# InternetMaximalism/plonky2_bn254

Hardware: AMD Instinct MI355X
Metric: G1 scalar-mul STARK proofs/sec (256-bit scalars) (higher is better)
Workload: dtype u64 (Goldilocks p = 2^64-2^32+1; BN254 Fq as 10x26-bit Montgomery limbs); 1 GPU; configs[1]: batch of 1024 G1 scalar-muls on 1 GPU per step = 8 proofs x 128 instances, 2^16 rows, W=781, standard_fast_config; instances_per_proof=128, steps_in_flight=4, parallelism=1 GPU, no collective

## Files before the change

### plonky2_bn254_amd/csrc/aux.h

```cpp
#pragma once
#include "gl_dev.h"
#include "../../include/bn254_stark.h"

static constexpr int CTL_MAX = 2, CTL_MAX_COLS = 160;

struct CtlSpecDev {
  int ncols[CTL_MAX];
  int filter_col[CTL_MAX];
  short col_start[CTL_MAX][CTL_MAX_COLS];
  unsigned char col_bits[CTL_MAX][CTL_MAX_COLS];
};

struct StarkShape {
  int W = 0;
  int rc_begin = 0, rc_end = 0;
  int table_col = 0, freq_col = 0;
  int n_ctl = 2;
  int n_constraints = 0;
  CtlSpecDev ctl;
  GL_HD int n_rc() const { return rc_end - rc_begin; }
  GL_HD int n_helpers() const { return (n_rc() + 1) / 2; }
  GL_HD int n_aux() const { return 2 * (n_helpers() + 1) + 2 * n_ctl; }
  GL_HD int n_lookup_cols() const { return 2 * (n_helpers() + 1); }
  GL_HD int n_total_constraints() const { return n_constraints + 2 * (n_helpers() + 2) + 2 * 2 * n_ctl; }
};

size_t aux_scratch_words(const StarkShape& sh, size_t N);
void aux_build(const StarkShape& sh, const u64* d_trace, size_t N, const u64 betas[2], const u64 gammas[2], u64* d_aux,
               u64* d_scratch, int* d_err, hipStream_t st);
```

### plonky2_bn254_amd/csrc/aux.hip

```cpp
#include <algorithm>
#include "aux.h"

static constexpr int LOGUP_SPAN = 16;
static constexpr int LOGUP_INV_BATCH = 4;

__global__ __launch_bounds__(256) void k_logup_inv_table(u64 beta0, u64 beta1, u64* __restrict__ inv) {
  const u32 t = blockIdx.x * blockDim.x + threadIdx.x;
  if (t >= 2 * 65536 / LOGUP_INV_BATCH) return;
  u64 d[LOGUP_INV_BATCH], pre[LOGUP_INV_BATCH];
  u64 acc = 1;
#pragma unroll
  for (int j = 0; j < LOGUP_INV_BATCH; j++) {
    const u64 x = gl_add((j & 1) ? beta1 : beta0, (u64)(2 * t + (j >> 1)));
    d[j] = x ? x : 1;
    pre[j] = acc;
    acc = gl_mul(acc, d[j]);
  }
  u64 r = gl_inv(acc);
  u64 o[LOGUP_INV_BATCH];
#pragma unroll
  for (int j = LOGUP_INV_BATCH - 1; j >= 0; j--) {
    const u64 x = gl_add((j & 1) ? beta1 : beta0, (u64)(2 * t + (j >> 1)));
    o[j] = x ? gl_mul(r, pre[j]) : 0;
    r = gl_mul(r, d[j]);
// ... 80 lines not shown
  part[t] = s;
  __syncthreads();
  for (int off = 1; off < T; off <<= 1) {
    u64 v = t >= off ? part[t - off] : 0;
    __syncthreads();
    part[t] = gl_add(part[t], v);
    __syncthreads();
  }
  u64 run = t ? part[t - 1] : 0;
  for (size_t q = 0; q < per; q++) {
    u64 x = src[idx(q0 + q)];
    if (mode == 0) {
      dst[idx(q0 + q)] = run;
      run = gl_add(run, x);
    } else {
      run = gl_add(run, x);
      dst[idx(q0 + q)] = run;
    }
  }
}

__global__ __launch_bounds__(256) void k_ctl_terms(const u64* __restrict__ trace, size_t N, CtlSpecDev spec, u64 beta0,
                                                   u64 gamma0, u64 beta1, u64 gamma1, u64* __restrict__ terms,
                                                   int* __restrict__ err) {
  const size_t i = (size_t)blockIdx.x * blockDim.x + threadIdx.x;
  if (i >= N) return;
  const int ctl = blockIdx.y;
  u64 f = trace[(size_t)spec.filter_col[ctl] * N + i];
  u64 t0 = 0, t1 = 0;
  if (f == 1) {
    u64 a0 = 0, a1 = 0;
    for (int m = spec.ncols[ctl] - 1; m >= 0; m--) {
      int start = spec.col_start[ctl][m], nb = spec.col_bits[ctl][m];
      u64 v = 0;
      for (int b = nb - 1; b >= 0; b--) v = gl_add(gl_dbl(v), trace[(size_t)(start + b) * N + i]);
      a0 = gl_add(gl_mul(a0, beta0), v);
      a1 = gl_add(gl_mul(a1, beta1), v);
    }
    t0 = gl_inv(gl_add(a0, gamma0));
    t1 = gl_inv(gl_add(a1, gamma1));
  } else if (f != 0) {
    atomicCAS(err, 0, BN254S_E_INTERNAL);
  }
  terms[(size_t)(ctl * 2 + 0) * N + i] = t0;
  terms[(size_t)(ctl * 2 + 1) * N + i] = t1;
}

static constexpr size_t LOGUP_INV_WORDS = 2 * 65536;
size_t aux_scratch_words(const StarkShape& sh, size_t N) {
  int nchunks = (sh.n_helpers() + LOGUP_SPAN - 1) / LOGUP_SPAN;
  return LOGUP_INV_WORDS + (size_t)(2 * nchunks + 2 + 2 * sh.n_ctl) * N;
}

void aux_build(const StarkShape& sh, const u64* d_trace, size_t N, const u64 betas[2], const u64 gammas[2], u64* d_aux,
               u64* d_scratch, int* d_err, hipStream_t st) {
  const int n_rc = sh.n_rc(), m = sh.n_helpers();
  const int nchunks = (m + LOGUP_SPAN - 1) / LOGUP_SPAN;
  u64* inv = d_scratch;
  u64* psum = inv + LOGUP_INV_WORDS;
  u64* terms = psum + (size_t)2 * nchunks * N;
  u64* cterms = terms + 2 * N;
  const unsigned scan_threads = (unsigned)std::min<size_t>(1024, N);
  k_logup_inv_table<<<(unsigned)(LOGUP_INV_WORDS / LOGUP_INV_BATCH / 256), 256, 0, st>>>(betas[0], betas[1], inv);
  dim3 g1((unsigned)((N + 255) / 256), nchunks);
  k_logup_helpers<<<g1, 256, 0, st>>>(d_trace, N, sh.rc_begin, n_rc, inv, d_aux, m, psum, nchunks, d_err);
  k_logup_terms<<<(unsigned)((N + 255) / 256), 256, 0, st>>>(d_trace, N, sh.table_col, sh.freq_col, inv, psum, nchunks, terms, d_err);
  k_scan<<<2, scan_threads, 0, st>>>(terms, N, d_aux + (size_t)m * N, (size_t)(m + 1) * N, N, 0);
  if (sh.n_ctl == 0) return;
  dim3 g3((unsigned)((N + 255) / 256), sh.n_ctl);
  k_ctl_terms<<<g3, 256, 0, st>>>(d_trace, N, sh.ctl, betas[0], gammas[0], betas[1], gammas[1], cterms, d_err);
  k_scan<<<2 * sh.n_ctl, scan_threads, 0, st>>>(cterms, N, d_aux + (size_t)2 * (m + 1) * N, N, N, 1);
}

void aux_module_warm() {
  hipFuncAttributes a;
  (void)hipFuncGetAttributes(&a, reinterpret_cast<const void*>(&k_logup_terms));
}
```

### plonky2_bn254_amd/csrc/ctx.h

```cpp
#pragma once
#include <string>
#include <vector>
#include <map>
#include <cstdio>
#include <mutex>
#include <condition_variable>
#include <chrono>
#include <deque>
#include <functional>
#include <thread>
#include <atomic>
#include <hip/hip_runtime.h>
#include "../../include/bn254_stark.h"
#include "gl_dev.h"
#include "ntt.h"

struct BufPool {
  std::map<std::string, std::pair<void*, size_t>> pool;
  std::string err;
  void* buf(const std::string& name, size_t bytes) {
    auto it = pool.find(name);
    if (it != pool.end() && it->second.second >= bytes) return it->second.first;
    if (it != pool.end()) {
      hipFree(it->second.first);
      pool.erase(it);
    }
    void* p = nullptr;
    if (hipMalloc(&p, bytes) != hipSuccess) {
      (void)hipGetLastError();
      err = "hipMalloc failed for " + name + " (" + std::to_string(bytes) + " bytes)";
      return nullptr;
    }
    pool[name] = {p, bytes};
    return p;
  }
  u64* words(const std::string& name, size_t n) { return (u64*)buf(name, n * 8); }
  bool has(const std::string& name) const { return pool.find(name) != pool.end(); }
  void drop(const std::string& name) {
    auto it = pool.find(name);
    if (it == pool.end()) return;
    hipFree(it->second.first);
    pool.erase(it);
  }
  void release() {
    for (auto& kv : pool) hipFree(kv.second.first);
    pool.clear();
  }
};

struct Slot {
  hipStream_t st = nullptr;
  BufPool mem;
  void* pinned = nullptr;
  size_t pinned_bytes = 0;
  std::vector<hipEvent_t> events;
};

// ... 75 lines not shown
    }
    cv.notify_all();
  }
  size_t active() {
    std::lock_guard<std::mutex> lk(mu);
    return n_busy - n_waiting;
  }
  size_t completions_now() {
    std::lock_guard<std::mutex> lk(mu);
    return completions;
  }
  void wait_for_a_completion(size_t c0) {
    std::unique_lock<std::mutex> lk(mu);
    n_waiting++;
    done_cv.wait_for(lk, std::chrono::seconds(60), [&] { return completions != c0; });
    n_waiting--;
  }
  void shutdown() {
    {
      std::lock_guard<std::mutex> lk(mu);
      stop = true;
    }
    cv.notify_all();
    for (auto& t : th) t.join();
    th.clear();
  }
};

struct bn254s_ctx : BufPool {
  int device = 0;
  hipStream_t stream = nullptr;
  NttTables ntt;
  std::vector<Slot*> slots;
  WorkPool workers;
  std::mutex plans_mu;
  std::map<std::pair<unsigned, bool>, NttPlan> plans;
  const NttPlan* ntt_plan(unsigned log_n, bool split) {
    std::lock_guard<std::mutex> lk(plans_mu);
    const auto key = std::make_pair(log_n, split);
    auto it = plans.find(key);
    if (it != plans.end()) return &it->second;
    NttPlan p;
    if (ntt_plan_init(&p, &ntt, log_n, split) != 0) return nullptr;
    return &(plans[key] = p);
  }
  std::mutex big_mu;
  std::condition_variable big_cv;
  int big_cap = 12, big_cost[4] = {12, 2, 4, 2}, big_used = 0;
  int hash_split = 1;
  bool big_fifo = true;
  struct BigWaiter {
    unsigned long id;
    int cls;
  };
  std::deque<BigWaiter> big_q;
  unsigned long big_next_id = 0;
  int big_convoy = 4, big_convoy_run = 0;
  bool big_last_was_ntt = false;
  void big_lock(int cls) {
    std::unique_lock<std::mutex> lk(big_mu);
    if (big_fifo) {
      const unsigned long my = big_next_id++;
      big_q.push_back({my, cls});
      big_cv.wait(lk, [&] {
        if (big_q.front().id == my) {
          if (big_used + big_cost[cls] > big_cap) return false;
          if (big_last_was_ntt && cls != BIG_NTT && big_convoy_run < big_convoy)
            for (const BigWaiter& w : big_q)
              if (w.cls == BIG_NTT) return false;
          return true;
        }
        if (cls != BIG_NTT || !big_last_was_ntt || big_used != 0 || big_convoy_run >= big_convoy) return false;
        if (big_q.front().cls == BIG_NTT) return false;
        for (const BigWaiter& w : big_q) {
          if (w.cls == BIG_NTT) return w.id == my;
        }
        return false;
      });
      const bool in_order = big_q.front().id == my;
      for (auto it = big_q.begin(); it != big_q.end(); ++it)
        if (it->id == my) {
          big_q.erase(it);
          break;
        }
      if (in_order) big_convoy_run = 0;
      else big_convoy_run++;
      big_last_was_ntt = false;
      big_used += big_cost[cls];
      lk.unlock();
      big_cv.notify_all();
      return;
    }
    big_cv.wait(lk, [&] { return big_used + big_cost[cls] <= big_cap; });
    big_used += big_cost[cls];
  }
  void big_unlock(int cls) {
    {
      std::lock_guard<std::mutex> lk(big_mu);
      big_used -= big_cost[cls];
      big_last_was_ntt = cls == BIG_NTT && big_used == 0;
    }
    big_cv.notify_all();
  }
  static constexpr size_t MAX_SLOTS = 64;
  std::mutex slots_mu, err_mu;
  float vb_ms[5] = {0, 0, 0, 0, 0};
  bn254s_ctx() { slots.reserve(MAX_SLOTS); }
  void set_err(const std::string& e) {
    std::lock_guard<std::mutex> lk(err_mu);
    err = e;
  }
  size_t n_slots_now() {
    std::lock_guard<std::mutex> lk(slots_mu);
    return slots.size();
  }
  Slot* slot(size_t i) {
    if (i >= MAX_SLOTS) return nullptr;
    std::lock_guard<std::mutex> lk(slots_mu);
    while (slots.size() <= i) {
      Slot* s = new Slot();
      if (hipStreamCreateWithFlags(&s->st, hipStreamNonBlocking) != hipSuccess) {
        delete s;
        return nullptr;
      }
      slots.push_back(s);
    }
    return slots[i];
  }
};

#define HIP_TRY(ctx, call)                                                                  \
  do {                                                                                      \
    hipError_t e_ = (call);                                                                 \
    if (e_ != hipSuccess) {                                                                 \
      (ctx)->set_err(std::string(#call) + ": " + hipGetErrorString(e_));                    \
      return BN254S_E_HIP;                                                                  \
    }                                                                                       \
  } while (0)
```

### plonky2_bn254_amd/csrc/prover.hip

```cpp
#include <algorithm>
#include <atomic>
#include <cstring>
#include <thread>
#include "ctx.h"
#include "trace.h"
#include "aux.h"
#include "merkle.h"
#include "quotient.h"
#include "fri.h"
#include "transcript.h"
#include "prover.h"
#include "proof_plan.h"
#include "transforms.h"

template <class L>
static StarkShape make_shape(bool input_has_a, int n_constraints) {
  StarkShape s;
  s.W = L::W;
  s.rc_begin = L::RC_BEGIN;
  s.rc_end = L::RC_END;
  s.table_col = L::RANGE;
  s.freq_col = L::FREQ;
  s.n_ctl = 2;
  s.n_constraints = n_constraints;
// ... 19 lines not shown
}
const StarkKind& stark_kind(int kind) {
  static const StarkKind kinds[3] = {
      {make_shape<G1L>(true, 1111), 8, true, g1_trace_scratch_words, g1_generate_trace_device, g1_quotient_mz_blocks, g1_quotient_launch},
      {make_shape<G2L>(true, 1693), 16, true, g2_trace_scratch_words, g2_generate_trace_device, g2_quotient_mz_blocks, g2_quotient_launch},
      {make_shape<FQL>(false, 770), 4, false, fq_trace_scratch_words, fq_generate_trace_no_offset, fq_quotient_mz_blocks, fq_quotient_launch}};
  return kinds[kind];
}

enum { ST_TRACE = 0, ST_TRACE_NTT, ST_TRACE_MERKLE, ST_AUX, ST_AUX_NTT, ST_AUX_MERKLE, ST_QUOTIENT, ST_QUOTIENT_COMMIT,
       ST_OPENINGS, ST_FRI, ST_TOTAL, ST_COUNT };
static const char* STAGE_NAMES[ST_COUNT] = {"trace_gen", "trace_ntt", "trace_merkle", "aux_columns", "aux_ntt", "aux_merkle",
                                            "quotient", "quotient_commit", "openings", "fri", "total"};

struct bn254s_proof {
  std::vector<u64> words, outputs;
  size_t sec_off[BN254S_SEC_COUNT + 1] = {0};
  int degree_bits = 0;
  float stage_ms[ST_COUNT] = {0};
};

std::vector<int> fri_arities(const bn254s_params& P, int degree_bits) {
  std::vector<int> a;
  int d = degree_bits;
  while (d > (int)P.final_poly_bits && d + (int)P.rate_bits - (int)P.arity_bits >= (int)P.cap_height) {
    a.push_back(P.arity_bits);
    d -= P.arity_bits;
  }
  return a;
}

__global__ __launch_bounds__(256) void k_quotient_chunks(const u64* __restrict__ ab, u64* __restrict__ out, size_t N, u64 inv2,
                                                         u64 inv2c) {
  size_t i = (size_t)blockIdx.x * blockDim.x + threadIdx.x;
  if (i >= N) return;
  int a = blockIdx.y;
  u64 A = ab[(size_t)(a * 2 + 0) * N + i], B = ab[(size_t)(a * 2 + 1) * N + i];
  out[(size_t)(a * 2 + 0) * N + i] = gl_mul(gl_add(A, B), inv2);
  out[(size_t)(a * 2 + 1) * N + i] = gl_mul(gl_sub(A, B), inv2c);
}

#define CHK(call)                                              \
  do {                                                         \
    hipError_t e_ = (call);                                    \
    if (e_ != hipSuccess) {                                    \
      err = std::string(#call) + ": " + hipGetErrorString(e_); \
      return BN254S_E_HIP;                                     \
    }                                                          \
  } while (0)

struct BigSection {
  bn254s_ctx* c;
  hipStream_t st;
  int cls;
  BigSection(bn254s_ctx* c_, hipStream_t st_, int cls_) : c(c_), st(st_), cls(cls_) { c->big_lock(cls); }
  ~BigSection() {
    hipStreamSynchronize(st);
    c->big_unlock(cls);
  }
};

static int get_point_tables(bn254s_ctx* c, unsigned log_n, QPointTables& pt) {
  static std::mutex mu;
  std::lock_guard<std::mutex> lk(mu);
  std::string key = "pt." + std::to_string(log_n);
  bool fresh = !c->has(key);
  size_t M2 = (size_t)2 << log_n;
  u64* p = c->words(key, 3 * M2);
  if (!p) return BN254S_E_OOM;
  if (fresh) {
    quotient_point_tables(p, p + M2, p + 2 * M2, log_n, c->stream);
    if (hipStreamSynchronize(c->stream) != hipSuccess) return BN254S_E_HIP;
  }
  pt.x = p;
  pt.lfirst = p + M2;
  pt.llast = p + 2 * M2;
  return 0;
}

struct Workspace {
  Slot* sl = nullptr;
  const ProofPlan* pl = nullptr;
  u64 *in, *tvals, *tcoef, *hist, *tmp, *ldechunk, *sponge, *comb, *tlde, *trees, *avals, *acoef, *alde, *scr, *quot, *tabs, *open,
      *fri, *fritrees, *qout;
  int* err;
  unsigned long long* pow;
  u32* qidx;
  u64 *ttree, *atree, *qtree;
  u64 *qv, *ab, *qcoef, *qlde, *qpart;
  u64 *W, *mzt, *apow;
  size_t cap_off;
  u64 *tw = nullptr, *aw = nullptr, *wpt = nullptr, *qrows = nullptr;
  int begin_windows(std::string& err);
};

static int workspace_acquire(Slot& sl, const ProofPlan& pl, Workspace& ws, std::string& err) {
  BufPool& mem = sl.mem;
  const PlanBuffers& b = pl.words;
  const bool stream = pl.stream, lowmem = pl.lowmem;
  ws.sl = &sl;
  ws.pl = &pl;
  if (lowmem) {
    mem.drop("acoef");
    mem.drop("alde");
  }
  ws.in = mem.words("in", b.in);
  ws.tvals = mem.words("tvals", b.tvals);
  ws.tcoef = mem.words("tcoef", b.tcoef);
  ws.hist = mem.words("hist", b.hist);
  ws.tmp = mem.words("tmp", b.tmp);
  mem.drop("win");
// ... 70 lines not shown
  CHK(hipStreamSynchronize(sl->st));
  mem.drop("tvals");
  tvals = nullptr;
  u64* win = mem.words("win", pl->words.win);
  if (!win) {
    err = mem.err;
    mem.release();
    return BN254S_E_OOM;
  }
  tw = win;
  aw = win + (size_t)pl->W * WROWS;
  wpt = aw + (size_t)pl->A * WROWS;
  qrows = wpt + 3 * WROWS;
  return BN254S_OK;
}

struct Run {
  bn254s_ctx* c;
  Slot& sl;
  hipStream_t st;
  const ProofPlan& pl;
  Workspace& ws;
  const Transforms& tf;
  QPointTables pt;
  void sb(int stage) const { hipEventRecord(sl.events[2 * stage], st); }
  void se(int stage) const { hipEventRecord(sl.events[2 * stage + 1], st); }
  int mmode() const { return c->workers.in_flight.load(std::memory_order_relaxed) >= 4 ? MERKLE_THROUGHPUT : MERKLE_LATENCY; }
};

static int upload_and_generate(const StarkKind& sk, const u64* scalars, const u64* x, const u64* off, size_t n, u64* d_in, u64* d_trace,
                               size_t N, u64* d_scr, u64* d_outs, int* d_err, hipStream_t st, bool with_range, std::string& err) {
  const size_t PW = sk.point_words;
  u64* d_sc = d_in;
  u64* d_x = d_in + 4 * n;
  u64* d_off = d_x + PW * n;
  CHK(hipMemcpyAsync(d_sc, scalars, n * 32, hipMemcpyHostToDevice, st));
  CHK(hipMemcpyAsync(d_x, x, n * PW * 8, hipMemcpyHostToDevice, st));
  if (sk.has_offset) CHK(hipMemcpyAsync(d_off, off, n * PW * 8, hipMemcpyHostToDevice, st));
  if (sk.generate_trace(d_sc, d_x, d_off, n, d_trace, N, d_scr, d_outs, d_err, st, with_range)) {
    err = "trace generation launch failed";
    return BN254S_E_HIP;
  }
  return BN254S_OK;
}

static int stage_trace(const Run& r, const u64* scalars, const u64* x, const u64* off, bn254s_proof* pr, int* h_err, std::string& err) {
  const ProofPlan& pl = r.pl;
  const Workspace& ws = r.ws;
  const StarkShape& sh = pl.sh;
  hipStream_t st = r.st;
  r.sb(ST_TRACE);
  CHK(hipMemsetAsync(ws.err, 0, 16, st));
  u64* d_outs = ws.open;
  if (int rc = upload_and_generate(stark_kind(pl.kind), scalars, x, off, pl.n, ws.in, ws.tvals, pl.N, ws.scr, d_outs, ws.err, st, false, err))
    return rc;
  {
    BigSection big(r.c, st, BIG_EXCL);
    launch_range_columns(ws.tvals, pl.N, sh.rc_begin, sh.rc_end, sh.freq_col, sh.table_col, (u32*)ws.hist, ws.err, st);
  }
  pr->outputs.resize(pl.n * (size_t)pl.PW);
  CHK(hipMemcpyAsync(pr->outputs.data(), d_outs, pl.n * (size_t)pl.PW * 8, hipMemcpyDeviceToHost, st));
  CHK(hipMemcpyAsync(h_err, ws.err, 4, hipMemcpyDeviceToHost, st));
  r.se(ST_TRACE);
  return BN254S_OK;
}

static void hash_sections(const Run& r, const u64* lde, int width, u64* tree, int stage) {
  bn254s_ctx* c = r.c;
  const size_t M2 = r.pl.M2;
  const int S = r.pl.log_n == 16 ? c->hash_split : 1;
  if (S <= 1) {
    BigSection big(c, r.st, BIG_HASH);
    r.sb(stage);
    merkle_leaves(lde, 1, M2, width, r.pl.log_m2, tree, r.st);
    return;
  }
  const size_t cnt = M2 / S;
  for (int k = 0; k < S; k++) {
    BigSection big(c, r.st, BIG_HASH_PART);
    if (k == 0) r.sb(stage);
    merkle_leaves_range(lde, 1, M2, width, (size_t)k * cnt, cnt, tree, r.st);
  }
}

static int commit(const Run& r, const u64* vals, u64* coef, u64* lde, int width, u64* tree, int ntt_stage, int merkle_stage,
                  u64* cap_out, std::string& err) {
  const ProofPlan& pl = r.pl;
  hipStream_t st = r.st;
  if (pl.stream) {
    BigSection big(r.c, st, BIG_NTT);
    r.sb(ntt_stage);
    r.tf.commit_stream(vals, coef, width, tree);
    r.se(ntt_stage);
    r.sb(merkle_stage);
  } else {
    {
      BigSection big(r.c, st, BIG_NTT);
      r.sb(ntt_stage);
      r.tf.commit_ntt(vals, coef, lde, width);
      r.se(ntt_stage);
    }
    hash_sections(r, lde, width, tree, merkle_stage);
  }
  merkle_upper(pl.log_m2, pl.P.cap_height, tree, st, r.mmode());
  CHK(hipMemcpyAsync(cap_out, tree + r.ws.cap_off, ProofPlan::CAPW * 8, hipMemcpyDeviceToHost, st));
  r.se(merkle_stage);
  CHK(hipStreamSynchronize(st));
  return BN254S_OK;
}

static void stage_aux(const Run& r, const u64 betas[2], const u64 gammas[2]) {
  BigSection big(r.c, r.st, BIG_EXCL);
  r.sb(ST_AUX);
  aux_build(r.pl.sh, r.ws.tvals, r.pl.N, betas, gammas, r.ws.avals, r.ws.scr, r.ws.err, r.st);
  r.se(ST_AUX);
}

static void quotient_over_windows(const Run& r, const u64 betas[2], const u64 gammas[2]) {
  const ProofPlan& pl = r.pl;
  const Workspace& ws = r.ws;
  hipStream_t st = r.st;
  const size_t N = pl.N, M2 = pl.M2, BK = pl.BK, WROWS = pl.WROWS;
  BigSection big(r.c, st, BIG_NTT);
  r.sb(ST_QUOTIENT);
  QPointTables wpt;
  wpt.x = ws.wpt;
  wpt.lfirst = ws.wpt + WROWS;
  wpt.llast = ws.wpt + 2 * WROWS;
  for (int h = 0; h < 2; h++)
    for (size_t k0 = 0; k0 < N; k0 += BK) {
      r.tf.for_lde_chunks(ws.tcoef, pl.W, 1 << h, [&](int c0, int cn) {
        fri_extract_window(ws.ldechunk, M2, pl.log_n, h, k0, WROWS, cn, ws.tw + (size_t)c0 * WROWS, st);
      });
      r.tf.for_lde_chunks(ws.acoef, pl.A, 1 << h, [&](int c0, int cn) {
        fri_extract_window(ws.ldechunk, M2, pl.log_n, h, k0, WROWS, cn, ws.aw + (size_t)c0 * WROWS, st);
      });
      quotient_point_tables_window(ws.wpt, ws.wpt + WROWS, ws.wpt + 2 * WROWS, pl.log_n, h, k0, WROWS, st);
      QArgs QA;
      quotient_fill_args(QA, pl.sh, nullptr, nullptr, ws.W, ws.mzt, r.pt, betas, gammas, pl.log_n, ws.qv, ws.qpart);
      quotient_window_args(QA, ws.tw, ws.aw, wpt, ws.qpart, WROWS, BK, k0, h);
      stark_kind(pl.kind).quotient_launch(QA, pl.sh, st);
    }
}

static int stage_quotient(const Run& r, const u64 alphas[2], const u64 betas[2], const u64 gammas[2], u64* cap_out, std::string& err) {
  const ProofPlan& pl = r.pl;
  const Workspace& ws = r.ws;
  const StarkKind& sk = stark_kind(pl.kind);
  hipStream_t st = r.st;
  const size_t N = pl.N;
  {
    std::vector<u64> hW, hmzt;
    const int* mz_e0 = nullptr;
    const int nblk = sk.mz_blocks(&mz_e0);
    quotient_host_tables(pl.K, alphas, mz_e0, nblk, hW, hmzt);
    CHK(hipMemcpyAsync(ws.W, hW.data(), hW.size() * 8, hipMemcpyHostToDevice, st));
    CHK(hipMemcpyAsync(ws.mzt, hmzt.data(), hmzt.size() * 8, hipMemcpyHostToDevice, st));
    CHK(hipStreamSynchronize(st));
  }
  if (pl.stream) {
    quotient_over_windows(r, betas, gammas);
  } else {
    BigSection big(r.c, st, BIG_EXCL);
    r.sb(ST_QUOTIENT);
    QArgs QA;
    quotient_fill_args(QA, pl.sh, ws.tlde, ws.alde, ws.W, ws.mzt, r.pt, betas, gammas, pl.log_n, ws.qv, ws.qpart);
    sk.quotient_launch(QA, pl.sh, st);
  }
  r.tf.quotient_coset_inverse(ws.qv, ws.ab);
  {
    u64 gn = gl_pow(GL_GEN, N);
    u64 inv2 = gl_inv(2), inv2c = gl_inv(gl_mul(2, gn));
    dim3 g((unsigned)((N + 255) / 256), 2);
    k_quotient_chunks<<<g, 256, 0, st>>>(ws.ab, ws.qcoef, N, inv2, inv2c);
  }
  r.se(ST_QUOTIENT);
  r.sb(ST_QUOTIENT_COMMIT);
  r.tf.lde(ws.qcoef, ws.qlde, ProofPlan::NQ);
  merkle_build(ws.qlde, 1, pl.M2, ProofPlan::NQ, pl.log_m2, pl.P.cap_height, ws.qtree, st, r.mmode());
  CHK(hipMemcpyAsync(cap_out, ws.qtree + ws.cap_off, ProofPlan::CAPW * 8, hipMemcpyDeviceToHost, st));
  r.se(ST_QUOTIENT_COMMIT);
  CHK(hipStreamSynchronize(st));
  return BN254S_OK;
}

static int stage_openings(const Run& r, gl2 zeta, gl2 zeta_next, u64* h_part, std::string& err) {
  const ProofPlan& pl = r.pl;
  const Workspace& ws = r.ws;
  hipStream_t st = r.st;
  const int W = pl.W, A = pl.A, NQ = ProofPlan::NQ, NSPL = pl.NSPL;
  const size_t R = pl.R, NH = pl.NH;
  {
    BigSection big(r.c, st, BIG_EXCL);
    r.sb(ST_OPENINGS);
    u64* d_otab = ws.open + pl.n_part();
    fri_opening_tables(pl.log_r, pl.log_s ? gl2_mul(zeta, zeta) : zeta, pl.log_s ? gl2_mul(zeta_next, zeta_next) : zeta_next, d_otab, st);
    fri_openings(ws.tcoef, NH, pl.log_r, W * NSPL, d_otab, ws.open, st);
    fri_openings(ws.acoef, NH, pl.log_r, A * NSPL, d_otab, ws.open + (size_t)W * NSPL * R * 5, st);
    fri_openings(ws.qcoef, NH, pl.log_r, NQ * NSPL, d_otab, ws.open + (size_t)(W + A) * NSPL * R * 5, st);
  }
  CHK(hipMemcpyAsync(h_part, ws.open, pl.n_part() * 8, hipMemcpyDeviceToHost, st));
  r.se(ST_OPENINGS);
  CHK(hipStreamSynchronize(st));
  return BN254S_OK;
}

static std::vector<u64> recombine_openings(const ProofPlan& pl, const u64* h_part, gl2 zeta, gl2 zeta_next) {
  const size_t R = pl.R;
  const int NSPL = pl.NSPL, n_polys = pl.W + pl.A + ProofPlan::NQ;
  std::vector<u64> h_open((size_t)n_polys * 5);
  std::vector<gl2> zp0(R), zp1(R);
  gl2 a = gl2_make(1, 0), b = gl2_make(1, 0);
  const gl2 y0 = pl.log_s ? gl2_mul(zeta, zeta) : zeta, y1 = pl.log_s ? gl2_mul(zeta_next, zeta_next) : zeta_next;
  for (size_t k1 = 0; k1 < R; k1++) {
    zp0[k1] = a;
    zp1[k1] = b;
    a = gl2_mul(a, y0);
    b = gl2_mul(b, y1);
  }
  for (int p = 0; p < n_polys; p++) {
    gl2 v0 = gl2_make(0, 0), v1 = gl2_make(0, 0);
    u64 s1 = 0;
    for (int half = 0; half < NSPL; half++) {
      gl2 e0 = gl2_make(0, 0), e1 = gl2_make(0, 0);
      for (size_t k1 = 0; k1 < R; k1++) {
        const u64* q = &h_part[(((size_t)p * NSPL + half) * R + k1) * 5];
        e0 = gl2_add(e0, gl2_mul(zp0[k1], gl2_make(q[0], q[1])));
        e1 = gl2_add(e1, gl2_mul(zp1[k1], gl2_make(q[2], q[3])));
        s1 = gl_add(s1, q[4]);
      }
      v0 = gl2_add(v0, half ? gl2_mul(zeta, e0) : e0);
      v1 = gl2_add(v1, half ? gl2_mul(zeta_next, e1) : e1);
    }
    u64* o5 = &h_open[(size_t)p * 5];
    o5[0] = v0.c0; o5[1] = v0.c1; o5[2] = v1.c0; o5[3] = v1.c1; o5[4] = s1;
  }
  return h_open;
}

struct Openings {
  const ProofPlan& pl;
  const std::vector<u64>& h_open;
  u64 operator()(int p, int k) const { return h_open[(size_t)p * 5 + k]; }
  int n_ctlz() const { return 2 * pl.sh.n_ctl; }
  u64 ctl_z_first(int i) const { return (*this)(pl.W + pl.sh.n_lookup_cols() + i, 4); }
};

static void observe_openings(Challenger& ch, const Openings& op) {
  const int W = op.pl.W, A = op.pl.A, NQ = ProofPlan::NQ;
  for (int p = 0; p < W + A + NQ; p++) {
    ch.observe(op(p, 0));
    ch.observe(op(p, 1));
  }
  for (int p = 0; p < W + A; p++) {
    ch.observe(op(p, 2));
    ch.observe(op(p, 3));
  }
  for (int i = 0; i < op.n_ctlz(); i++) {
    ch.observe(op.ctl_z_first(i));
    ch.observe(0);
  }
}

struct FriAlphaPowers {
  std::vector<u32> apow;
  gl2 r0, r1, r2;
};
static FriAlphaPowers fri_alpha_powers(const Openings& op, gl2 fri_alpha) {
  const int W = op.pl.W, A = op.pl.A, NQ = ProofPlan::NQ, n_ctlz = op.n_ctlz();
  FriAlphaPowers f;
  f.apow.assign(8 * (size_t)(W + A + NQ), 0);
  gl2 ap = gl2_make(1, 0);
  f.r0 = f.r1 = f.r2 = gl2_make(0, 0);
  for (int p = 0; p < W + A + NQ; p++) {
    fri_weight_record(&f.apow[8 * (size_t)p], ap);
    f.r0 = gl2_add(f.r0, gl2_mul(ap, gl2_make(op(p, 0), op(p, 1))));
    if (p < W + A) f.r1 = gl2_add(f.r1, gl2_mul(ap, gl2_make(op(p, 2), op(p, 3))));
    if (p < n_ctlz) f.r2 = gl2_add(f.r2, gl2_mul_base(ap, op.ctl_z_first(p)));
    ap = gl2_mul(ap, fri_alpha);
  }
  return f;
}

static int stage_fri_combine(const Run& r, const FriAlphaPowers& f, gl2 zeta, gl2 zeta_next, gl2 fri_alpha, std::string& err) {
  const ProofPlan& pl = r.pl;
  const Workspace& ws = r.ws;
  hipStream_t st = r.st;
  CHK(hipMemcpyAsync(ws.apow, f.apow.data(), f.apow.size() * 4, hipMemcpyHostToDevice, st));
  CHK(hipStreamSynchronize(st));
  BigSection big(r.c, st, BIG_EXCL);
  r.sb(ST_FRI);
  fri_combine_coeffs(pl.sh, ws.tcoef, ws.acoef, ws.qcoef, ws.apow, pl.N, ws.comb, st);
  r.tf.lde(ws.comb, ws.comb + (size_t)6 * pl.N, 6);
  fri_combine_final(pl.sh, ws.comb + (size_t)6 * pl.N, r.pt.x, zeta, zeta_next, f.r0, f.r1, f.r2, fri_alpha, pl.M2, ws.fri, st);
  return BN254S_OK;
}

struct FriLayers {
  std::vector<std::vector<u64>> caps;
  std::vector<const u64*> vals, trees;
  const u64* last = nullptr;
  u64 shift = GL_GEN;
  unsigned lm = 0;
};

static int stage_fri_commit(const Run& r, Challenger& ch, FriLayers& fl, std::string& err) {
  const ProofPlan& pl = r.pl;
  hipStream_t st = r.st;
  const int L = pl.L, CAPW = ProofPlan::CAPW;
  fl.caps.assign(L, std::vector<u64>(CAPW));
  fl.vals.resize(L);
  fl.trees.resize(L);
  u64* vals = r.ws.fri;
  u64* ftree = r.ws.fritrees;
  fl.shift = GL_GEN;
  unsigned lm = pl.log_m2;
  const u64 inv16 = gl_inv(16);
  for (int l = 0; l < L; l++) {
    const int lg = (int)lm - 4;
    merkle_build(vals, 32, 1, 32, lg, pl.P.cap_height, ftree, st, r.mmode());
    CHK(hipMemcpyAsync(fl.caps[l].data(), ftree + 4 * merkle_level_offset(lg, lg - pl.P.cap_height), CAPW * 8,
                       hipMemcpyDeviceToHost, st));
    CHK(hipStreamSynchronize(st));
    ch.observe_n(fl.caps[l].data(), CAPW);
    gl2 beta = ch.challenge_ext();
    u64* next = vals + 2 * ((size_t)1 << lm);
    fri_fold(vals, next, lm, fl.shift, beta, inv16, st);
    fl.vals[l] = vals;
    fl.trees[l] = ftree;
    ftree += merkle_tree_digests(lg, pl.P.cap_height) * 4;
    vals = next;
    fl.shift = gl_pow(fl.shift, 16);
    lm -= 4;
  }
  fl.last = vals;
  fl.lm = lm;
  return BN254S_OK;
}

static int fri_final_poly(const std::vector<u64>& h_final, unsigned lm, u64 shift, unsigned rate_bits, std::vector<gl2>& final_poly,
                          std::string& err) {
  const size_t Mf = (size_t)1 << lm;
  final_poly.assign(Mf >> rate_bits, gl2_make(0, 0));
// ... 139 lines not shown
  mark(BN254S_SEC_INIT_CHALLENGER_STATE);
  o.insert(o.end(), pp.init_state, pp.init_state + 12);
  mark(BN254S_SEC_COUNT);
  pr->degree_bits = pl.log_n;
}

static int prove_on_slot(bn254s_ctx* c, Slot& sl, int kind, const bn254s_params& P, const u64* scalars, const u64* x,
                         const u64* off, size_t n, bn254s_proof* pr, std::string& err,
                         const std::function<void()>* after_alloc = nullptr) {
  size_t dev_free_b = 0, dev_total_b = 0;
  (void)hipMemGetInfo(&dev_free_b, &dev_total_b);
  ProofPlan pl;
  if (int rc = proof_plan(kind, n, P, dev_total_b, plan_overrides_from_env(), pl, err)) return rc;
  hipStream_t st = sl.st;
  QPointTables pt;
  if (int rc = get_point_tables(c, pl.log_n, pt)) {
    err = "point tables";
    return rc;
  }
  const NttPlan* np = c->ntt_plan(pl.log_n, pl.log_s != 0);
  if (!np) {
    err = "NTT tables";
    return BN254S_E_OOM;
  }
  Workspace ws;
  if (int rc = workspace_acquire(sl, pl, ws, err)) return rc;
  if (after_alloc) (*after_alloc)();
  const Transforms tf{*np, st, pl, ws.tmp, ws.ldechunk, ws.sponge};
  if (sl.events.empty()) {
    sl.events.resize(2 * ST_COUNT);
    for (auto& e : sl.events) CHK(hipEventCreate(&e));
  }
  const Run r{c, sl, st, pl, ws, tf, pt};
  const int CAPW = ProofPlan::CAPW;
  ProofParts pp;
  Challenger ch;

  r.sb(ST_TOTAL);
  int h_err = 0;
  if (int rc = stage_trace(r, scalars, x, off, pr, &h_err, err)) return rc;
  if (int rc = commit(r, ws.tvals, ws.tcoef, ws.tlde, pl.W, ws.ttree, ST_TRACE_NTT, ST_TRACE_MERKLE, pp.caps[0], err)) return rc;
  if (h_err) {
    err = "trace generation reported device error " + std::to_string(h_err);
    return h_err;
  }
  ch.observe_n(pp.caps[0], CAPW);
  u64 betas[2], gammas[2];
  for (int i = 0; i < 2; i++) {
    betas[i] = ch.challenge();
    gammas[i] = ch.challenge();
  }
  ch.compact(pp.init_state);

  stage_aux(r, betas, gammas);
  if (pl.stream)
    if (int rc = ws.begin_windows(err)) return rc;
  if (int rc = commit(r, ws.avals, ws.acoef, ws.alde, pl.A, ws.atree, ST_AUX_NTT, ST_AUX_MERKLE, pp.caps[1], err)) return rc;
  ch.observe_n(pp.caps[1], CAPW);
  u64 alphas[2] = {ch.challenge(), 0};
  alphas[1] = ch.challenge();

  if (int rc = stage_quotient(r, alphas, betas, gammas, pp.caps[2], err)) return rc;
  ch.observe_n(pp.caps[2], CAPW);
  gl2 zeta = ch.challenge_ext();
  {
    gl2 zp = zeta;
    for (unsigned i = 0; i < pl.log_n; i++) zp = gl2_mul(zp, zp);
    if (gl2_eq(zp, gl2_make(1, 0))) {
      err = "Opening point is in the subgroup.";
      return BN254S_E_TRANSCRIPT;
    }
  }
  const gl2 zeta_next = gl2_mul_base(zeta, gl_root_of_unity(pl.log_n));

  u64* staging = (u64*)sl.pinned;
  if (int rc = stage_openings(r, zeta, zeta_next, staging, err)) return rc;
  pp.h_open = recombine_openings(pl, staging, zeta, zeta_next);
  const Openings op{pl, pp.h_open};
  observe_openings(ch, op);

  const gl2 fri_alpha = ch.challenge_ext();
  if (int rc = stage_fri_combine(r, fri_alpha_powers(op, fri_alpha), zeta, zeta_next, fri_alpha, err)) return rc;
  if (int rc = stage_fri_commit(r, ch, pp.fri, err)) return rc;
  std::vector<u64> h_final((size_t)2 << pp.fri.lm);
  CHK(hipMemcpyAsync(h_final.data(), pp.fri.last, h_final.size() * 8, hipMemcpyDeviceToHost, st));
  CHK(hipStreamSynchronize(st));
  if (int rc = fri_final_poly(h_final, pp.fri.lm, pp.fri.shift, P.rate_bits, pp.final_poly, err)) return rc;
  for (auto& cf : pp.final_poly) {
    ch.observe(cf.c0);
    ch.observe(cf.c1);
  }
  if (int rc = stage_pow(r, ch, pp.pow_witness, err)) return rc;
  pp.h_q = staging;
  if (int rc = stage_queries(r, ch, pp.fri, staging, err)) return rc;

  assemble_proof(pl, pp, pr);
  for (int i = 0; i < ST_COUNT; i++) hipEventElapsedTime(&pr->stage_ms[i], sl.events[2 * i], sl.events[2 * i + 1]);
  return BN254S_OK;
}

extern "C" {

struct bn254s_batch {
  bn254s_ctx* c = nullptr;
  int kind = 0;
  bn254s_params params;
  const u64 *scalars = nullptr, *x = nullptr, *off = nullptr;
// ... 265 lines not shown
```

### plonky2_bn254_amd/csrc/trace.h

```cpp
#pragma once
#include "gl_dev.h"
#include "layout.h"
#include "../../include/bn254_stark.h"

size_t g1_trace_scratch_words(size_t n);
size_t g2_trace_scratch_words(size_t n);
size_t fq_trace_scratch_words(size_t n);
int g1_generate_trace_device(const u64* d_scalars, const u64* d_x, const u64* d_off, size_t n, u64* d_trace, size_t N,
                             u64* d_scratch, u64* d_outputs, int* d_err, hipStream_t st, bool with_range = true);
int g2_generate_trace_device(const u64* d_scalars, const u64* d_x, const u64* d_off, size_t n, u64* d_trace, size_t N,
                             u64* d_scratch, u64* d_outputs, int* d_err, hipStream_t st, bool with_range = true);
int fq_generate_trace_device(const u64* d_scalars, const u64* d_x, size_t n, u64* d_trace, size_t N, u64* d_scratch,
                             u64* d_outputs, int* d_err, hipStream_t st, bool with_range = true);

void launch_g1_dbl_chain(const u64* d_x, int n, u64* px, u64* py, u64* pz, hipStream_t st);
void launch_g2_dbl_chain(const u64* d_x, int n, u64* pts, u64* znorm, hipStream_t st);

void launch_fq_batch_inv(const u64* in, u64* out, size_t count, hipStream_t st);
void launch_round_flag_table(u64* tbl, hipStream_t st);
void launch_range_columns(u64* trace, size_t N, int rc_begin, int rc_end, int freq_col, int range_col, u32* hist, int* err,
                          hipStream_t st);
void launch_fq_inv_selftest(const u64* in, u64* out, size_t n, hipStream_t st);
```

### plonky2_bn254_amd/csrc/trace_shared.hip

```cpp
#include "trace_common.h"
#include "trace.h"

#ifndef BN254S_BATCH_INV_CH
#define BN254S_BATCH_INV_CH 4
#endif
template <int J, int CH>
__device__ __forceinline__ void batch_inv_back(const fq (&v)[CH], const fq (&pre)[CH], fq& inv, u64* __restrict__ out, size_t count,
                                               size_t tid, size_t T) {
  if constexpr (J >= 0) {
    const size_t e = tid + J * T;
    if (e < count) {
      if (fq_is_zero(v[J])) {
        st_fq(out, count, e, fq_zero());
      } else {
        st_fq(out, count, e, fq_mul(inv, pre[J]));
        if constexpr (J > 0) inv = fq_mul(inv, v[J]);
      }
    }
    batch_inv_back<J - 1, CH>(v, pre, inv, out, count, tid, T);
  }
}
template <int CH>
__global__ __launch_bounds__(64) void k_fq_batch_inv(const u64* __restrict__ in, u64* __restrict__ out, size_t count) {
  LATENCY_KERNEL_PRIO();
// ... 36 lines not shown
    u64 v = i < hi ? src[i] : ~0ULL;
    if (i < hi && v >= 65536) atomicCAS(err, 0, BN254S_E_INTERNAL);
    bool active = i < hi && (v >> 15) == half;
    u32 bin = (u32)v & 32767;
#pragma unroll
    for (int r = 0; r < 2; r++) {
      unsigned long long m = __ballot(active);
      if (m == 0) break;
      int leader = __ffsll((long long)m) - 1;
      u32 lv = __shfl(bin, leader);
      bool same = active && bin == lv;
      unsigned long long ms = __ballot(same);
      if (lane == leader) atomicAdd(&h[lv], (u32)__popcll(ms));
      active = active && !same;
    }
    if (active) atomicAdd(&h[bin], 1u);
  }
  __syncthreads();
  for (int b = threadIdx.x; b < 32768; b += blockDim.x) {
    u32 cnt = h[b];
    if (cnt) atomicAdd(&hist[half * 32768 + b], cnt);
  }
}
__global__ __launch_bounds__(256) void k_range_columns(u64* __restrict__ trace, size_t N, int freq_col, int range_col,
                                                       const u32* __restrict__ hist) {
  LATENCY_KERNEL_PRIO();
  size_t i = (size_t)blockIdx.x * blockDim.x + threadIdx.x;
  if (i >= N) return;
  trace[(size_t)range_col * N + i] = i < 65536 ? i : 65535;
  trace[(size_t)freq_col * N + i] = i < 65536 ? (u64)hist[i] : 0;
}

__global__ __launch_bounds__(64) void k_fq_inv_selftest(const u64* __restrict__ in, u64* __restrict__ out, size_t n) {
  size_t i = (size_t)blockIdx.x * blockDim.x + threadIdx.x;
  if (i >= n) return;
  const fq a = fq_from_canonical(in + 4 * i);
  const bool z = fq_is_zero(a);
  const fqw r0 = fq_to_canonical(z ? a : fq_inv(a)), r1 = fq_to_canonical(z ? a : fq_inv_fermat(a));
  for (int k = 0; k < 4; k++) {
    out[8 * i + k] = r0.l[k];
    out[8 * i + 4 + k] = r1.l[k];
  }
}
void launch_fq_inv_selftest(const u64* in, u64* out, size_t n, hipStream_t st) {
  k_fq_inv_selftest<<<(unsigned)((n + 63) / 64), 64, 0, st>>>(in, out, n);
}

void launch_fq_batch_inv(const u64* in, u64* out, size_t count, hipStream_t st) {
  const int CH = BN254S_BATCH_INV_CH;
  size_t threads = (count + CH - 1) / CH;
  k_fq_batch_inv<CH><<<(unsigned)((threads + 63) / 64), 64, 0, st>>>(in, out, count);
}
void launch_round_flag_table(u64* tbl, hipStream_t st) { k_round_flag_table<<<2, 256, 0, st>>>(tbl); }
void launch_range_columns(u64* trace, size_t N, int rc_begin, int rc_end, int freq_col, int range_col, u32* hist, int* err,
                          hipStream_t st) {
  hipMemsetAsync(hist, 0, 65536 * 4, st);
  k_histogram<<<dim3(128, 2), 1024, 0, st>>>(trace, N, rc_begin, rc_end, hist, err);
  k_range_columns<<<(unsigned)((N + 255) / 256), 256, 0, st>>>(trace, N, freq_col, range_col, hist);
}

void trace_shared_module_warm() {
  hipFuncAttributes a;
  (void)hipFuncGetAttributes(&a, reinterpret_cast<const void*>(&k_range_columns));
}
```

Measured before the change: 91.21 proofs/s.

## Shrink exclusive GPU sections and reserve admission tickets before trace generation

The aux build is split into wide kernels, which stay inside the exclusive big-section lock, and the latency-bound scans, which now run after the lock is released. The range-fill kernel is likewise moved out of the exclusive section. A ticket is reserved in the FIFO admission queue before trace generation, so the later exclusive request keeps its place, and NTT waiters defer to tickets that are not yet asking. The aim is to shorten how long each proof holds exclusive admission so concurrent steps overlap better. This adds stream syncs after trace generation and after aux, and an optional env-gated admission log.

Result: no change. 91.89 proofs/s (median of 6 runs) (+0.7%).

```diff
diff --git a/plonky2_bn254_amd/csrc/aux.h b/plonky2_bn254_amd/csrc/aux.h
--- a/plonky2_bn254_amd/csrc/aux.h
+++ b/plonky2_bn254_amd/csrc/aux.h
@@ -28,3 +28,6 @@
 size_t aux_scratch_words(const StarkShape& sh, size_t N);
 void aux_build(const StarkShape& sh, const u64* d_trace, size_t N, const u64 betas[2], const u64 gammas[2], u64* d_aux,
                u64* d_scratch, int* d_err, hipStream_t st);
+void aux_build_wide(const StarkShape& sh, const u64* d_trace, size_t N, const u64 betas[2], const u64 gammas[2], u64* d_aux,
+                    u64* d_scratch, int* d_err, hipStream_t st);
+void aux_build_scans(const StarkShape& sh, size_t N, u64* d_aux, u64* d_scratch, hipStream_t st);
diff --git a/plonky2_bn254_amd/csrc/aux.hip b/plonky2_bn254_amd/csrc/aux.hip
--- a/plonky2_bn254_amd/csrc/aux.hip
+++ b/plonky2_bn254_amd/csrc/aux.hip
@@ -156,24 +156,45 @@
   return LOGUP_INV_WORDS + (size_t)(2 * nchunks + 2 + 2 * sh.n_ctl) * N;
 }
 
+struct AuxScratch {
+  int nchunks;
+  u64 *inv, *psum, *terms, *cterms;
+  AuxScratch(const StarkShape& sh, size_t N, u64* d_scratch) {
+    nchunks = (sh.n_helpers() + LOGUP_SPAN - 1) / LOGUP_SPAN;
+    inv = d_scratch;
+    psum = inv + LOGUP_INV_WORDS;
+    terms = psum + (size_t)2 * nchunks * N;
+    cterms = terms + 2 * N;
+  }
+};
+
+void aux_build_wide(const StarkShape& sh, const u64* d_trace, size_t N, const u64 betas[2], const u64 gammas[2], u64* d_aux,
+                    u64* d_scratch, int* d_err, hipStream_t st) {
+  const int n_rc = sh.n_rc(), m = sh.n_helpers();
+  const AuxScratch s(sh, N, d_scratch);
+  k_logup_inv_table<<<(unsigned)(LOGUP_INV_WORDS / LOGUP_INV_BATCH / 256), 256, 0, st>>>(betas[0], betas[1], s.inv);
+  dim3 g1((unsigned)((N + 255) / 256), s.nchunks);
+  k_logup_helpers<<<g1, 256, 0, st>>>(d_trace, N, sh.rc_begin, n_rc, s.inv, d_aux, m, s.psum, s.nchunks, d_err);
+  k_logup_terms<<<(unsigned)((N + 255) / 256), 256, 0, st>>>(d_trace, N, sh.table_col, sh.freq_col, s.inv, s.psum, s.nchunks, s.terms,
+                                                             d_err);
+  if (sh.n_ctl == 0) return;
+  dim3 g3((unsigned)((N + 255) / 256), sh.n_ctl);
+  k_ctl_terms<<<g3, 256, 0, st>>>(d_trace, N, sh.ctl, betas[0], gammas[0], betas[1], gammas[1], s.cterms, d_err);
+}
+
+void aux_build_scans(const StarkShape& sh, size_t N, u64* d_aux, u64* d_scratch, hipStream_t st) {
+  const int m = sh.n_helpers();
+  const AuxScratch s(sh, N, d_scratch);
+  const unsigned scan_threads = (unsigned)std::min<size_t>(1024, N);
+  k_scan<<<2, scan_threads, 0, st>>>(s.terms, N, d_aux + (size_t)m * N, (size_t)(m + 1) * N, N, 0);
+  if (sh.n_ctl == 0) return;
+  k_scan<<<2 * sh.n_ctl, scan_threads, 0, st>>>(s.cterms, N, d_aux + (size_t)2 * (m + 1) * N, N, N, 1);
+}
+
 void aux_build(const StarkShape& sh, const u64* d_trace, size_t N, const u64 betas[2], const u64 gammas[2], u64* d_aux,
                u64* d_scratch, int* d_err, hipStream_t st) {
-  const int n_rc = sh.n_rc(), m = sh.n_helpers();
-  const int nchunks = (m + LOGUP_SPAN - 1) / LOGUP_SPAN;
-  u64* inv = d_scratch;
-  u64* psum = inv + LOGUP_INV_WORDS;
-  u64* terms = psum + (size_t)2 * nchunks * N;
-  u64* cterms = terms + 2 * N;
-  const unsigned scan_threads = (unsigned)std::min<size_t>(1024, N);
-  k_logup_inv_table<<<(unsigned)(LOGUP_INV_WORDS / LOGUP_INV_BATCH / 256), 256, 0, st>>>(betas[0], betas[1], inv);
-  dim3 g1((unsigned)((N + 255) / 256), nchunks);
-  k_logup_helpers<<<g1, 256, 0, st>>>(d_trace, N, sh.rc_begin, n_rc, inv, d_aux, m, psum, nchunks, d_err);
-  k_logup_terms<<<(unsigned)((N + 255) / 256), 256, 0, st>>>(d_trace, N, sh.table_col, sh.freq_col, inv, psum, nchunks, terms, d_err);
-  k_scan<<<2, scan_threads, 0, st>>>(terms, N, d_aux + (size_t)m * N, (size_t)(m + 1) * N, N, 0);
-  if (sh.n_ctl == 0) return;
-  dim3 g3((unsigned)((N + 255) / 256), sh.n_ctl);
-  k_ctl_terms<<<g3, 256, 0, st>>>(d_trace, N, sh.ctl, betas[0], gammas[0], betas[1], gammas[1], cterms, d_err);
-  k_scan<<<2 * sh.n_ctl, scan_threads, 0, st>>>(cterms, N, d_aux + (size_t)2 * (m + 1) * N, N, N, 1);
+  aux_build_wide(sh, d_trace, N, betas, gammas, d_aux, d_scratch, d_err, st);
+  aux_build_scans(sh, N, d_aux, d_scratch, st);
 }
 
 void aux_module_warm() {
diff --git a/plonky2_bn254_amd/csrc/ctx.h b/plonky2_bn254_amd/csrc/ctx.h
--- a/plonky2_bn254_amd/csrc/ctx.h
+++ b/plonky2_bn254_amd/csrc/ctx.h
@@ -3,6 +3,7 @@
 #include <vector>
 #include <map>
 #include <cstdio>
+#include <cstdlib>
 #include <mutex>
 #include <condition_variable>
 #include <chrono>
@@ -184,18 +185,55 @@
   struct BigWaiter {
     unsigned long id;
     int cls;
+    bool asking;
   };
   std::deque<BigWaiter> big_q;
   unsigned long big_next_id = 0;
   int big_convoy = 4, big_convoy_run = 0;
   bool big_last_was_ntt = false;
-  void big_lock(int cls) {
+  static constexpr unsigned long NO_TICKET = ~0ul;
+  unsigned long big_reserve(int cls) {
+    std::lock_guard<std::mutex> lk(big_mu);
+    if (!big_fifo) return NO_TICKET;
+    big_q.push_back({big_next_id, cls, false});
+    return big_next_id++;
+  }
+  void big_cancel(unsigned long ticket) {
+    if (ticket == NO_TICKET) return;
+    {
+      std::lock_guard<std::mutex> lk(big_mu);
+      for (auto it = big_q.begin(); it != big_q.end(); ++it)
+        if (it->id == ticket) {
+          big_q.erase(it);
+          break;
+        }
+    }
+    big_cv.notify_all();
+  }
+  void big_lock(int cls, unsigned long ticket = NO_TICKET) {
     std::unique_lock<std::mutex> lk(big_mu);
     if (big_fifo) {
-      const unsigned long my = big_next_id++;
-      big_q.push_back({my, cls});
+      unsigned long my = ticket;
+      if (ticket == NO_TICKET) {
+        my = big_next_id++;
+        big_q.push_back({my, cls, true});
+      } else {
+        for (BigWaiter& w : big_q)
+          if (w.id == my) w.asking = true;
+        big_cv.notify_all();
+      }
+      auto head = [&]() -> const BigWaiter& {
+        for (const BigWaiter& w : big_q)
+          if (w.asking) return w;
+        return big_q.front();
+      };
       big_cv.wait(lk, [&] {
-        if (big_q.front().id == my) {
+        if (cls == BIG_NTT)
+          for (const BigWaiter& w : big_q) {
+            if (w.id == my) break;
+            if (!w.asking) return false;
+          }
+        if (head().id == my) {
           if (big_used + big_cost[cls] > big_cap) return false;
           if (big_last_was_ntt && cls != BIG_NTT && big_convoy_run < big_convoy)
             for (const BigWaiter& w : big_q)
@@ -203,13 +241,13 @@
           return true;
         }
         if (cls != BIG_NTT || !big_last_was_ntt || big_used != 0 || big_convoy_run >= big_convoy) return false;
-        if (big_q.front().cls == BIG_NTT) return false;
+        if (head().cls == BIG_NTT) return false;
         for (const BigWaiter& w : big_q) {
           if (w.cls == BIG_NTT) return w.id == my;
         }
         return false;
       });
-      const bool in_order = big_q.front().id == my;
+      const bool in_order = head().id == my;
       for (auto it = big_q.begin(); it != big_q.end(); ++it)
         if (it->id == my) {
           big_q.erase(it);
@@ -237,7 +275,23 @@
   static constexpr size_t MAX_SLOTS = 64;
   std::mutex slots_mu, err_mu;
   float vb_ms[5] = {0, 0, 0, 0, 0};
-  bn254s_ctx() { slots.reserve(MAX_SLOTS); }
+  FILE* adm_log = nullptr;
+  std::mutex adm_mu;
+  std::chrono::steady_clock::time_point adm_t0 = std::chrono::steady_clock::now();
+  double adm_now_ms() const { return std::chrono::duration<double, std::milli>(std::chrono::steady_clock::now() - adm_t0).count(); }
+  void adm_record(const char* cls, const char* stage, int cost, double at_ms, double lead_ms, double tail_ms, double held_ms) {
+    std::lock_guard<std::mutex> lk(adm_mu);
+    fprintf(adm_log, "%s %s %d %.3f %.4f %.4f %.4f\n", cls, stage, cost, at_ms, lead_ms, tail_ms, held_ms);
+    fflush(adm_log);
+  }
+  bn254s_ctx() {
+    slots.reserve(MAX_SLOTS);
+    if (const char* e = getenv("BN254S_ADMISSION_LOG"))
+      if (*e) adm_log = fopen(e, "a");
+  }
+  ~bn254s_ctx() {
+    if (adm_log) fclose(adm_log);
+  }
   void set_err(const std::string& e) {
     std::lock_guard<std::mutex> lk(err_mu);
     err = e;
diff --git a/plonky2_bn254_amd/csrc/prover.hip b/plonky2_bn254_amd/csrc/prover.hip
--- a/plonky2_bn254_amd/csrc/prover.hip
+++ b/plonky2_bn254_amd/csrc/prover.hip
@@ -95,11 +95,42 @@
 struct BigSection {
   bn254s_ctx* c;
   hipStream_t st;
-  int cls;
-  BigSection(bn254s_ctx* c_, hipStream_t st_, int cls_) : c(c_), st(st_), cls(cls_) { c->big_lock(cls); }
+  int cls, stage;
+  double at_ms = 0, lead_ms = 0;
+  hipEvent_t ev_wide = nullptr, ev_end = nullptr;
+  bool marked = false;
+  BigSection(bn254s_ctx* c_, hipStream_t st_, int cls_, int stage_, unsigned long ticket = bn254s_ctx::NO_TICKET)
+      : c(c_), st(st_), cls(cls_), stage(stage_) {
+    c->big_lock(cls, ticket);
+    if (c->adm_log) {
+      at_ms = c->adm_now_ms();
+      hipStreamSynchronize(st);
+      lead_ms = c->adm_now_ms() - at_ms;
+      hipEventCreate(&ev_wide);
+      hipEventCreate(&ev_end);
+    }
+  }
+  void wide_done() {
+    if (c->adm_log && !marked) {
+      hipEventRecord(ev_wide, st);
+      marked = true;
+    }
+  }
   ~BigSection() {
+    if (c->adm_log) {
+      wide_done();
+      hipEventRecord(ev_end, st);
+    }
     hipStreamSynchronize(st);
     c->big_unlock(cls);
+    if (c->adm_log) {
+      static const char* CLS[4] = {"ntt", "excl", "hash", "hash_part"};
+      float tail_ms = 0;
+      hipEventElapsedTime(&tail_ms, ev_wide, ev_end);
+      c->adm_record(CLS[cls], STAGE_NAMES[stage], c->big_cost[cls], at_ms, lead_ms, tail_ms, c->adm_now_ms() - at_ms);
+      hipEventDestroy(ev_wide);
+      hipEventDestroy(ev_end);
+    }
   }
 };
 
@@ -276,12 +307,21 @@
   r.sb(ST_TRACE);
   CHK(hipMemsetAsync(ws.err, 0, 16, st));
   u64* d_outs = ws.open;
-  if (int rc = upload_and_generate(stark_kind(pl.kind), scalars, x, off, pl.n, ws.in, ws.tvals, pl.N, ws.scr, d_outs, ws.err, st, false, err))
+  const unsigned long ticket = r.c->big_reserve(BIG_EXCL);
+  int rc = upload_and_generate(stark_kind(pl.kind), scalars, x, off, pl.n, ws.in, ws.tvals, pl.N, ws.scr, d_outs, ws.err, st, false, err);
+  if (rc == BN254S_OK && hipStreamSynchronize(st) != hipSuccess) {
+    err = "trace generation: the stream failed";
+    rc = BN254S_E_HIP;
+  }
+  if (rc) {
+    r.c->big_cancel(ticket);
     return rc;
+  }
   {
-    BigSection big(r.c, st, BIG_EXCL);
-    launch_range_columns(ws.tvals, pl.N, sh.rc_begin, sh.rc_end, sh.freq_col, sh.table_col, (u32*)ws.hist, ws.err, st);
-  }
+    BigSection big(r.c, st, BIG_EXCL, ST_TRACE, ticket);
+    launch_range_histogram(ws.tvals, pl.N, sh.rc_begin, sh.rc_end, (u32*)ws.hist, ws.err, st);
+  }
+  launch_range_fill(ws.tvals, pl.N, sh.freq_col, sh.table_col, (u32*)ws.hist, st);
   pr->outputs.resize(pl.n * (size_t)pl.PW);
   CHK(hipMemcpyAsync(pr->outputs.data(), d_outs, pl.n * (size_t)pl.PW * 8, hipMemcpyDeviceToHost, st));
   CHK(hipMemcpyAsync(h_err, ws.err, 4, hipMemcpyDeviceToHost, st));
@@ -294,14 +334,14 @@
   const size_t M2 = r.pl.M2;
   const int S = r.pl.log_n == 16 ? c->hash_split : 1;
   if (S <= 1) {
-    BigSection big(c, r.st, BIG_HASH);
+    BigSection big(c, r.st, BIG_HASH, stage);
     r.sb(stage);
     merkle_leaves(lde, 1, M2, width, r.pl.log_m2, tree, r.st);
     return;
   }
   const size_t cnt = M2 / S;
   for (int k = 0; k < S; k++) {
-    BigSection big(c, r.st, BIG_HASH_PART);
+    BigSection big(c, r.st, BIG_HASH_PART, stage);
     if (k == 0) r.sb(stage);
     merkle_leaves_range(lde, 1, M2, width, (size_t)k * cnt, cnt, tree, r.st);
   }
@@ -312,14 +352,14 @@
   const ProofPlan& pl = r.pl;
   hipStream_t st = r.st;
   if (pl.stream) {
-    BigSection big(r.c, st, BIG_NTT);
+    BigSection big(r.c, st, BIG_NTT, ntt_stage);
     r.sb(ntt_stage);
     r.tf.commit_stream(vals, coef, width, tree);
     r.se(ntt_stage);
     r.sb(merkle_stage);
   } else {
     {
-      BigSection big(r.c, st, BIG_NTT);
+      BigSection big(r.c, st, BIG_NTT, ntt_stage);
       r.sb(ntt_stage);
       r.tf.commit_ntt(vals, coef, lde, width);
       r.se(ntt_stage);
@@ -333,11 +373,16 @@
   return BN254S_OK;
 }
 
-static void stage_aux(const Run& r, const u64 betas[2], const u64 gammas[2]) {
-  BigSection big(r.c, r.st, BIG_EXCL);
-  r.sb(ST_AUX);
-  aux_build(r.pl.sh, r.ws.tvals, r.pl.N, betas, gammas, r.ws.avals, r.ws.scr, r.ws.err, r.st);
+static int stage_aux(const Run& r, const u64 betas[2], const u64 gammas[2], std::string& err) {
+  {
+    BigSection big(r.c, r.st, BIG_EXCL, ST_AUX);
+    r.sb(ST_AUX);
+    aux_build_wide(r.pl.sh, r.ws.tvals, r.pl.N, betas, gammas, r.ws.avals, r.ws.scr, r.ws.err, r.st);
+  }
+  aux_build_scans(r.pl.sh, r.pl.N, r.ws.avals, r.ws.scr, r.st);
   r.se(ST_AUX);
+  CHK(hipStreamSynchronize(r.st));
+  return BN254S_OK;
 }
 
 static void quotient_over_windows(const Run& r, const u64 betas[2], const u64 gammas[2]) {
@@ -345,7 +390,7 @@
   const Workspace& ws = r.ws;
   hipStream_t st = r.st;
   const size_t N = pl.N, M2 = pl.M2, BK = pl.BK, WROWS = pl.WROWS;
-  BigSection big(r.c, st, BIG_NTT);
+  BigSection big(r.c, st, BIG_NTT, ST_QUOTIENT);
   r.sb(ST_QUOTIENT);
   QPointTables wpt;
   wpt.x = ws.wpt;
@@ -385,7 +430,7 @@
   if (pl.stream) {
     quotient_over_windows(r, betas, gammas);
   } else {
-    BigSection big(r.c, st, BIG_EXCL);
+    BigSection big(r.c, st, BIG_EXCL, ST_QUOTIENT);
     r.sb(ST_QUOTIENT);
     QArgs QA;
     quotient_fill_args(QA, pl.sh, ws.tlde, ws.alde, ws.W, ws.mzt, r.pt, betas, gammas, pl.log_n, ws.qv, ws.qpart);
@@ -415,7 +460,7 @@
   const int W = pl.W, A = pl.A, NQ = ProofPlan::NQ, NSPL = pl.NSPL;
   const size_t R = pl.R, NH = pl.NH;
   {
-    BigSection big(r.c, st, BIG_EXCL);
+    BigSection big(r.c, st, BIG_EXCL, ST_OPENINGS);
     r.sb(ST_OPENINGS);
     u64* d_otab = ws.open + pl.n_part();
     fri_opening_tables(pl.log_r, pl.log_s ? gl2_mul(zeta, zeta) : zeta, pl.log_s ? gl2_mul(zeta_next, zeta_next) : zeta_next, d_otab, st);
@@ -512,7 +557,7 @@
   hipStream_t st = r.st;
   CHK(hipMemcpyAsync(ws.apow, f.apow.data(), f.apow.size() * 4, hipMemcpyHostToDevice, st));
   CHK(hipStreamSynchronize(st));
-  BigSection big(r.c, st, BIG_EXCL);
+  BigSection big(r.c, st, BIG_EXCL, ST_FRI);
   r.sb(ST_FRI);
   fri_combine_coeffs(pl.sh, ws.tcoef, ws.acoef, ws.qcoef, ws.apow, pl.N, ws.comb, st);
   r.tf.lde(ws.comb, ws.comb + (size_t)6 * pl.N, 6);
@@ -758,7 +803,7 @@
   }
   ch.compact(pp.init_state);
 
-  stage_aux(r, betas, gammas);
+  if (int rc = stage_aux(r, betas, gammas, err)) return rc;
   if (pl.stream)
     if (int rc = ws.begin_windows(err)) return rc;
   if (int rc = commit(r, ws.avals, ws.acoef, ws.alde, pl.A, ws.atree, ST_AUX_NTT, ST_AUX_MERKLE, pp.caps[1], err)) return rc;
diff --git a/plonky2_bn254_amd/csrc/trace.h b/plonky2_bn254_amd/csrc/trace.h
--- a/plonky2_bn254_amd/csrc/trace.h
+++ b/plonky2_bn254_amd/csrc/trace.h
@@ -20,4 +20,6 @@
 void launch_round_flag_table(u64* tbl, hipStream_t st);
 void launch_range_columns(u64* trace, size_t N, int rc_begin, int rc_end, int freq_col, int range_col, u32* hist, int* err,
                           hipStream_t st);
+void launch_range_histogram(const u64* trace, size_t N, int rc_begin, int rc_end, u32* hist, int* err, hipStream_t st);
+void launch_range_fill(u64* trace, size_t N, int freq_col, int range_col, const u32* hist, hipStream_t st);
 void launch_fq_inv_selftest(const u64* in, u64* out, size_t n, hipStream_t st);
diff --git a/plonky2_bn254_amd/csrc/trace_shared.hip b/plonky2_bn254_amd/csrc/trace_shared.hip
--- a/plonky2_bn254_amd/csrc/trace_shared.hip
+++ b/plonky2_bn254_amd/csrc/trace_shared.hip
@@ -112,11 +112,17 @@
   k_fq_batch_inv<CH><<<(unsigned)((threads + 63) / 64), 64, 0, st>>>(in, out, count);
 }
 void launch_round_flag_table(u64* tbl, hipStream_t st) { k_round_flag_table<<<2, 256, 0, st>>>(tbl); }
+void launch_range_histogram(const u64* trace, size_t N, int rc_begin, int rc_end, u32* hist, int* err, hipStream_t st) {
+  hipMemsetAsync(hist, 0, 65536 * 4, st);
+  k_histogram<<<dim3(128, 2), 1024, 0, st>>>(trace, N, rc_begin, rc_end, hist, err);
+}
+void launch_range_fill(u64* trace, size_t N, int freq_col, int range_col, const u32* hist, hipStream_t st) {
+  k_range_columns<<<(unsigned)((N + 255) / 256), 256, 0, st>>>(trace, N, freq_col, range_col, hist);
+}
 void launch_range_columns(u64* trace, size_t N, int rc_begin, int rc_end, int freq_col, int range_col, u32* hist, int* err,
                           hipStream_t st) {
-  hipMemsetAsync(hist, 0, 65536 * 4, st);
-  k_histogram<<<dim3(128, 2), 1024, 0, st>>>(trace, N, rc_begin, rc_end, hist, err);
-  k_range_columns<<<(unsigned)((N + 255) / 256), 256, 0, st>>>(trace, N, freq_col, range_col, hist);
+  launch_range_histogram(trace, N, rc_begin, rc_end, hist, err, st);
+  launch_range_fill(trace, N, freq_col, range_col, hist, st);
 }
 
 void trace_shared_module_warm() {
```
